# ningchungui/dbscan-on-spark

Measured on AMD Instinct MI355X. Metric: points clustered/sec (whole node) at 1/2/4/8 MI355X; % HBM roofline, higher is better.
Workload: dtype f64; 1 GPU; config 2: G(10000000 points, 32 Gaussian blobs, noise=0.0, dense=1.0, seed=1), eps=2.55, minPoints=10, LocalDBSCANNaive semantics; n_points=10000000, min_points=10, parallelism=single GPU, one local fit, world_size=1, clusters=14396, core_points=8854960, occupied_cells=1447458, occupied_tiles=44430

## Files before the change

dbscan-on-spark_amd/csrc/fit.hip:

```cpp
#include "internal.h"

#include <cmath>
#include <cstdio>
#include <cstdlib>
#include <cstring>
#include <vector>

namespace dbscan {

enum GridMode { kGridEps = 0, kGridAllPairs = 1, kGridNoPairs = 2 };

namespace {

constexpr int kTslot = 65;
constexpr int kQReg = 4;
constexpr int64_t kTileGrid = 8192;
constexpr int kMaxNbr = 11;
constexpr int32_t kModeArcheryBox = 2;
constexpr int64_t kBoxEdgeCap = 1 << 20;

#ifndef DBSCAN_AB_STAMPS
#define DBSCAN_AB_STAMPS 0
#endif
#if DBSCAN_AB_STAMPS
// ... 1319 lines not shown
                int ex = 0;
#pragma unroll
                for (int s = 4; s > 0; s >>= 1)
                    if (ex + s < 8 && st.off[base + ex + s] <= j) ex += s;
                const int p = st.cb[base + ex] + (j - st.off[base + ex]);
                const bool is_core =
                    min_points <= 0 || count_point<true>(st, buf, xy, cell, seg, j, r * 8 + ex, p,
                                                         eps2, min_points, lst, nbr, nbr_k);
                parent[p] = p;
                core[p] = is_core ? 1 : 0;
                mine += is_core ? 1 : 0;
            }
        } else {
            for (int p = st.ts + (int)threadIdx.x; p < st.te; p += kBlock) {
                const bool is_core =
                    min_points <= 0 || count_point<false>(st, buf, xy, cell, seg, 0, 0, p, eps2,
                                                          min_points, lst, nbr, nbr_k);
                parent[p] = p;
                core[p] = is_core ? 1 : 0;
                mine += is_core ? 1 : 0;
            }
        }
        __syncthreads();
    }
    for (int o = 32; o > 0; o >>= 1) mine += __shfl_xor(mine, o, 64);
    if (__lane_id() == 0) wcores[threadIdx.x >> 6] = mine;
    __syncthreads();
    if (threadIdx.x == 0) {
        int tot = 0;
        for (int w = 0; w < kBlock / 64; ++w) tot += wcores[w];
        block_cores[blockIdx.x] = tot;
    }
}

struct F32Cut {
    float lo, hi;
    float ne2;
};

__device__ __forceinline__ F32Cut f32_cut(const GridParams& g, double eps2) {
    const double s = 0.5 * g.invx;
    const double e2 = eps2 * s * s;
    return {__double2float_rd(e2 - 0x1p-14), __double2float_ru(e2 + 0x1p-14), -(float)e2};
}

constexpr float kCountBand = 0x1p-14f;
typedef float pk2f __attribute__((ext_vector_type(2)));
__device__ __forceinline__ float count_d(float2 me, float2 q, float ne2) {
    const pk2f d = pk2f{q.x, q.y} - pk2f{me.x, me.y};
    return __builtin_fmaf(d.x, d.x, __builtin_fmaf(d.y, d.y, ne2));
}

__device__ __forceinline__ int stage_slot(const TileStage& st, int q) {
    int k = 0;
#pragma unroll
    for (int s = 64; s > 0; s >>= 1)
        if (k + s < 100 && st.off[k + s] <= q) k += s;
    return st.cb[k] + (q - st.off[k]);
}

__device__ __forceinline__ float f32_d2(float2 a, float2 b) {
    const float dx = b.x - a.x, dy = b.y - a.y;
    return __builtin_fmaf(dx, dx, dy * dy);
}

template <int CAP>
__device__ bool stage_build32(const StageMeta& m, const double2* __restrict__ xy, TileStage& st,
                              float2* buf, const GridParams& g, const TileOrg& o) {
    const int tid = threadIdx.x;
    if (tid < 100) {
        st.cb[tid] = m.b;
        st.cn[tid] = m.cnt;
    }
    if (tid == 0) {
        st.ts = m.ts;
        st.te = m.te;
        st.q0 = m.q0;
        st.nq = m.q1 - m.q0;
    }
    __syncthreads();
    if (tid < 64) {
        int carry = 0;
        for (int base = 0; base < 100; base += 64) {
            const int i = base + tid;
            const int v = i < 100 ? st.cn[i] : 0;
            int incl = v;
#pragma unroll
            for (int o = 1; o < 64; o <<= 1) {
                const int u = __shfl_up(incl, o, 64);
                if (tid >= o) incl += u;
            }
            if (i < 100) st.off[i] = carry + incl - v;
            carry += __shfl(incl, 63, 64);
        }
        if (tid == 0) {
            st.off[100] = carry;
            st.total = carry;
            st.ok = carry <= CAP;
        }
    }
    __syncthreads();
    if (st.ok) {
        constexpr int kPer = (CAP + kBlock - 1) / kBlock;
        const int total = st.total;
#pragma unroll
        for (int u = 0; u < kPer; ++u) {
            const int i = tid + u * kBlock;
            if (i < total) {
                int lo = 0;
#pragma unroll
                for (int s = 64; s > 0; s >>= 1)
                    if (lo + s < 100 && st.off[lo + s] <= i) lo += s;
                const double2 v = xy[st.cb[lo] + (i - st.off[lo])];
                buf[i] = make_float2((float)((v.x * 0.5 - o.xmin2) * g.invx - o.ox),
                                     (float)((v.y * 0.5 - o.ymin2) * g.invy - o.oy));
            }
        }
    }
    __syncthreads();
    return st.ok;
}

template <class CoreF, class ExactF>
__device__ __forceinline__ bool quarters_touch32(const float2* __restrict__ buf, int ab, int ae,
                                                 uint32_t am, int bb, int be, uint32_t bm,
                                                 CoreF is_core, F32Cut cut, ExactF exact) {
    if (ae - ab <= 32 && be - bb <= 32) {
        for (uint32_t m1 = am; m1; m1 &= m1 - 1) {
            const int ia = ab + __ffs(m1) - 1;
            const float2 pa = buf[ia];
            for (uint32_t m2 = bm; m2; m2 &= m2 - 1) {
                const int ib = bb + __ffs(m2) - 1;
                const float F = f32_d2(pa, buf[ib]);
                if (F <= cut.lo) return true;
                if (F <= cut.hi && exact(ia, ib)) return true;
            }
        }
        return false;
    }
    for (int i = ab; i < ae; ++i) {
        if (!is_core(i)) continue;
        const float2 pa = buf[i];
        for (int j = bb; j < be; ++j) {
            if (!is_core(j)) continue;
            const float F = f32_d2(pa, buf[j]);
            if (F <= cut.lo) return true;
            if (F <= cut.hi && exact(i, j)) return true;
        }
    }
    return false;
}


template <class CoreF, class ExactF>
__device__ __forceinline__ void unite_adjacent32(int* lp, const uint32_t* lrange,
                                                 const uint32_t* lmask, const uint16_t* qmap,
                                                 int qi, const float2* __restrict__ buf,
                                                 CoreF is_core, F32Cut cut, ExactF exact) {
    constexpr int kDx[4] = {-1, 0, 1, -1}, kDy[4] = {-1, -1, -1, 0};
    const uint32_t ri = lrange[qi], am = lmask[qi];
    const int lq = (int)((ri >> 22) & 255u);
    const int ab = (int)(ri & 2047u), ae = ab + (int)((ri >> 11) & 2047u);
    int jn[4];
#pragma unroll
    for (int o = 0; o < 4; ++o) {
        const int ux = (lq & 15) + kDx[o], uy = (lq >> 4) + kDy[o];
        jn[o] = (ux >= 0 && ux <= 15 && uy >= 0) ? (int)qmap[uy * 16 + ux] : 0xFFFF;
    }
    uint32_t rj[4], mj[4];
#pragma unroll
    for (int o = 0; o < 4; ++o) {
        const int jj = jn[o] == 0xFFFF ? qi : jn[o];
        rj[o] = jn[o] == 0xFFFF ? 0u : lrange[jj];
        mj[o] = lmask[jj];
    }
    const float2 pa = buf[ab + (am ? __ffs(am) - 1 : 0)];
    bool t[4];
#pragma unroll
    for (int o = 0; o < 4; ++o) {
        const float2 pb = buf[(int)(rj[o] & 2047u) + (mj[o] ? __ffs(mj[o]) - 1 : 0)];
        t[o] = (rj[o] >> 31) && am && mj[o] && f32_d2(pa, pb) <= cut.lo;
    }
#pragma unroll
    for (int o = 0; o < 4; ++o) {
        if ((rj[o] >> 31) && !t[o]) {
            const int bb = (int)(rj[o] & 2047u), be = bb + (int)((rj[o] >> 11) & 2047u);
            t[o] = quarters_touch32(buf, ab, ae, am, bb, be, mj[o], is_core, cut, exact);
        }
        if (t[o]) lunite(lp, qi, jn[o]);
    }
}

constexpr int kScanBatch = 4;
template <bool REC, int STRIDE = kBlock, class ExactF>
__device__ __forceinline__ bool scan_count32(const float2* __restrict__ buf, int b, int e,
                                             float2 me, F32Cut cut, int min_points, int& cnt,
                                             uint32_t* lst, int& nrec, int nbr_k, int tag,
                                             ExactF exact, int* nbatch = nullptr) {
    for (int j = b; j < e; j += kScanBatch) {
        if (nbatch) ++*nbatch;
        const int nin = e - j;
        float2 qq[kScanBatch];
#pragma unroll
        for (int u = 0; u < kScanBatch; ++u) qq[u] = buf[j + u];
        const uint32_t valid = nin >= kScanBatch ? (1u << kScanBatch) - 1u : (1u << nin) - 1u;
        uint32_t hm = 0, am = 0;
        float d[kScanBatch];
#pragma unroll
        for (int u = 0; u < kScanBatch; ++u) d[u] = count_d(me, qq[u], cut.ne2);
#pragma unroll
        for (int u = kScanBatch - 1; u >= 0; --u)
            hm = __builtin_amdgcn_alignbit(hm, __float_as_uint(d[u]), 31);
        hm &= valid;
        float mn = fabsf(d[0]);
#pragma unroll
        for (int u = 1; u < kScanBatch; ++u) mn = fminf(mn, fabsf(d[u]));
        if (__builtin_expect(mn <= kCountBand, 0)) {
#pragma unroll
            for (int u = 0; u < kScanBatch; ++u)
                if (((valid >> u) & 1u) && fabsf(d[u]) <= kCountBand) am |= 1u << u;
            hm &= ~am;
        }
        if (__builtin_expect(am != 0, 0)) {
            for (uint32_t m = am; m; m &= m - 1) {
                const int u = __ffs(m) - 1;
                if (exact(j + u)) hm |= 1u << u;
            }
        }
        if (REC && hm && nrec < nbr_k) {
            lst[nrec * STRIDE] = (uint32_t)j | ((uint32_t)tag << 11) | (hm << 16);
            ++nrec;
        }
        cnt += __popc(hm);
        if (cnt >= min_points) return true;
    }
    return cnt >= min_points;
}

__device__ void fused_tile_union32(int t, int q0, int nq, int b, int e, uint32_t key,
                                   const FuseArgs& fa,
                                   const GridParams& g, const TileStage& st,
                                   const float2* __restrict__ buf,
                                   const uint32_t* __restrict__ lcore,
                                   const double2* __restrict__ xy, double eps2, F32Cut cut,
                                   int32_t* __restrict__ parent, UnionLds& u) {
    const int i = threadIdx.x;
    const auto is_core = [&](int j) { return ((lcore[j >> 5] >> (j & 31)) & 1u) != 0; };
    const auto exact = [&](int qa, int qb) {
        const double2 pa = xy[stage_slot(st, qa)], pb = xy[stage_slot(st, qb)];
        return within_eps(pa.x, pa.y, pb.x, pb.y, eps2);
    };
    __shared__ int s_first;
    __shared__ int s_tflags;
    if (i == 0) {
        s_first = 0x7FFFFFFF;
        s_tflags = 0;
    }
    u.qmap[i] = 0xFFFF;
    u.cmin[i] = ~0ull;
    lds_barrier();
    int rep = -1, best = 0x7FFFFFFF, gx = 0, gy = 0;
    if (i < nq) {
        uint32_t cx, cy;
        cell_xy(key >> 2, g.ntx, cx, cy);
        gx = (int)(2 * cx + (key & 1u));
        gy = (int)(2 * cy + ((key >> 1) & 1u));
        const int lq = (gy & 15) * 16 + (gx & 15);
        const int len = e - b;
        const int l = (int)((key >> 2) & 63u);
        const int k = ((l >> 3) + 1) * 10 + (l & 7) + 1;
        const int jb = st.off[k] + (b - st.cb[k]);
        uint32_t mask = 0;
        int first = -1;
        if (len <= 32) {
            const int w = jb >> 5, o = jb & 31;
            const uint64_t v = (uint64_t)lcore[w] | ((uint64_t)lcore[w + 1] << 32);
            mask = (uint32_t)(v >> o) & (len == 32 ? ~0u : ((1u << len) - 1u));
            first = mask ? __ffs(mask) - 1 : -1;
        } else {
            for (int j = 0; j < len && (j < 32 || first < 0); ++j)
                if (is_core(jb + j)) {
                    if (j < 32) mask |= 1u << j;
                    if (first < 0) first = j;
                }
        }
        if (first >= 0) {
            rep = b + first;
            best = fa.perm[rep];
        }
        if (rep >= 0) {
            atomicMin(&s_first, i);
            const int tf = ((gx & 15) >= 14 ? 1 : 0) | ((gy & 15) >= 14 ? 2 : 0);
            if (tf) atomicOr(&s_tflags, tf);
        }
        fa.qinfo[q0 + i] = make_int4(b, e, rep, (int)mask);
        u.lp[i] = i;
        u.lrange[i] = (rep >= 0 ? 0x80000000u : 0u) | ((uint32_t)lq << 22) | (uint32_t)jb |
                      ((uint32_t)len << 11);
        u.lmask[i] = mask;
        u.qmap[lq] = (uint16_t)i;
    }
    lds_barrier();
    if (i == 0) fa.tcore[t] = (uint8_t)s_tflags;
    AB_STAMP(5);
    {
        if (i < nq && rep >= 0)
            unite_adjacent32(u.lp, u.lrange, u.lmask, u.qmap, i, buf, is_core, cut, exact);
        lds_barrier();
        AB_STAMP(6);
        const int f = s_first;
        const bool split = i < nq && rep >= 0 && lfind(u.lp, i) != lfind(u.lp, f);
        if (__syncthreads_or(split)) {
            for (int k = i; k < nq * 8; k += kBlock) {
                const int o = k / nq, qi = k - o * nq;
                const uint32_t ri = u.lrange[qi];
                if (!(ri >> 31)) continue;
                const int lq = (int)((ri >> 22) & 255u);
                const int ux = (lq & 15) + kRingDx[4 + o], uy = (lq >> 4) + kRingDy[4 + o];
                if (ux < 0 || uy < 0 || ux > 15 || uy > 15) continue;
                const int j = u.qmap[uy * 16 + ux];
                if (j == 0xFFFF) continue;
                const uint32_t rj = u.lrange[j];
                if (!(rj >> 31)) continue;
                if (lfind(u.lp, qi) == lfind(u.lp, j)) continue;
                const int ab = (int)(ri & 2047u), ae = ab + (int)((ri >> 11) & 2047u);
                const int bb = (int)(rj & 2047u), be = bb + (int)((rj >> 11) & 2047u);
                if (quarters_touch32(buf, ab, ae, u.lmask[qi], bb, be, u.lmask[j], is_core, cut,
                                     exact))
                    lunite(u.lp, qi, j);
            }
            lds_barrier();
        }
        AB_STAMP(7);
    }
    int r = -1;
    if (i < nq && rep >= 0) {
        r = lfind(u.lp, i);
        atomicMin(&u.cmin[r], ((unsigned long long)(uint32_t)best << 32) | (uint32_t)rep);
    }
    lds_barrier();
    AB_STAMP(8);
    if (i < nq) {
        const int crep = r >= 0 ? (int)(uint32_t)(u.cmin[r] & 0xFFFFFFFFull) : -1;
        fa.qg[q0 + i] = make_int4(gx, gy, best, 0);
        fa.qcomp[q0 + i] = crep;
        if (rep >= 0) parent[rep] = crep;
    }
}

template <int CAP, int MINW>
__global__ __launch_bounds__(kBlock, MINW) void count_tile32_kernel(
    const double2* __restrict__ xy, const int32_t* __restrict__ tstart,
    const int2* __restrict__ tstage, const int32_t* __restrict__ ntiles_p, double eps2,
    int32_t min_points, uint8_t* __restrict__ core, int32_t* __restrict__ parent,
    int32_t* __restrict__ block_cores, int32_t* __restrict__ nbr, int nbr_k, FuseArgs fa) {
    const GridParams g = *fa.gp;
    if (!g.clique) {
        if (threadIdx.x == 0) block_cores[blockIdx.x] = 0;
        return;
    }
    __shared__ TileStage st;
    __shared__ float2 buf[CAP + kScanBatch];
    __shared__ int wcores[kBlock / 64];
    __shared__ int rowoff[9];
    __shared__ __attribute__((aligned(16))) uint32_t lsts[kMaxNbr * kBlock];
    __shared__ uint32_t lcore[(CAP + 31) / 32 + 1];
    static_assert(CAP < 2048, "LDS ranges are packed in 11 bits");
    static_assert(sizeof(UnionLds) <= sizeof(lsts), "UnionLds must fit");
    uint32_t* lst = lsts + threadIdx.x;
    const int ntiles = *ntiles_p;
    const F32Cut cut = f32_cut(g, eps2);
    int mine = 0;
    const BucketWalk<kMedBuckets> order(fa.tl.mb);
    const int nt = order.size();
    const auto tile_at = [&](int k) { return k < nt ? order.at(fa.tl.medium, fa.tl.cap, k) : ntiles; };
    StageMeta meta = stage_meta(tile_at(blockIdx.x), ntiles, tstage, tstart, fa.tq);
    for (int k = blockIdx.x; k < nt; k += gridDim.x) {
        AB_STAMP(0);
        const int t = tile_at(k);
        if (threadIdx.x < (CAP + 31) / 32 + 1) lcore[threadIdx.x] = 0u;
        stage_build32<CAP>(meta, xy, st, buf, g, tile_org(g, fa.tpart, t, fa.tkey[t]));
        AB_STAMP(1);
        AB_NOTE(10, st.total);
        meta = stage_meta(tile_at(k + gridDim.x), ntiles, tstage, tstart, fa.tq);
        const int q0 = st.q0, nq = st.nq;
        int qb = 0, qe = 0;
        uint32_t qk = 0;
        if ((int)threadIdx.x < nq) {
            qb = fa.qstart[q0 + threadIdx.x];
            qe = fa.qstart[q0 + threadIdx.x + 1];
            qk = fa.qkey[q0 + threadIdx.x];
        }
        {
            if (threadIdx.x == 0) {
                int acc = 0;
                for (int r = 0; r < 8; ++r) {
                    rowoff[r] = acc;
                    acc += st.off[(r + 1) * 10 + 9] - st.off[(r + 1) * 10 + 1];
                }
                rowoff[8] = acc;
            }
            __syncthreads();
            AB_STAMP(2);
            const int own = rowoff[8];
            AB_NOTE(11, own);
            for (int i = (int)threadIdx.x; i < own; i += kBlock) {
                int r = 0;
#pragma unroll
                for (int s = 4; s > 0; s >>= 1)
                    if (r + s < 8 && rowoff[r + s] <= i) r += s;
                const int base = (r + 1) * 10 + 1;
                const int j = st.off[base] + (i - rowoff[r]);
                int ex = 0;
#pragma unroll
                for (int s = 4; s > 0; s >>= 1)
                    if (ex + s < 8 && st.off[base + ex + s] <= j) ex += s;
                const int p = st.cb[base + ex] + (j - st.off[base + ex]);
                bool is_core = true;
                if (min_points > 0) {
                    const int l = r * 8 + ex;
                    const float2 me = buf[j];
                    const LdsRanges rg = lds_ranges(st, l);
                    const auto exact = [&](int q) {
                        const double2 a = xy[p], o = xy[stage_slot(st, q)];
                        return within_eps(a.x, a.y, o.x, o.y, eps2);
                    };
                    int cnt = 0, nrec = 0;
                    const int k_rec = nbr_k;
#if DBSCAN_AB_COUNTDIV
                    int nbt = 0;
                    int* const nbp = &nbt;
#else
                    int* const nbp = nullptr;
#endif
                    bool done = scan_count32<true>(buf, rg.cs, rg.ce, me, cut, min_points, cnt,
                                                   lst, nrec, k_rec, 0, exact, nbp);
#pragma unroll
                    for (int k = 0; k < 3 && !done; ++k) {
                        const int lo = rg.b[k], hi = rg.e[k];
                        if (lo <= rg.cs && rg.ce <= hi) {
                            done = scan_count32<true>(buf, lo, rg.cs, me, cut, min_points, cnt,
                                                      lst, nrec, k_rec, k, exact, nbp) ||
                                   scan_count32<true>(buf, rg.ce, hi, me, cut, min_points, cnt,
                                                      lst, nrec, k_rec, k, exact, nbp);
                        } else {
                            done = scan_count32<true>(buf, lo, hi, me, cut, min_points, cnt, lst,
                                                      nrec, k_rec, k, exact, nbp);
                        }
                    }
                    is_core = cnt >= min_points;
#if DBSCAN_AB_COUNTDIV
                    {
                        const uint64_t act = __ballot(1);
                        int mx = nbt, sm = nbt;
                        for (int o = 32; o > 0; o >>= 1) {
                            mx = max(mx, __shfl_xor(mx, o, 64));
                            sm += __shfl_xor(sm, o, 64);
                        }
                        const uint64_t cm = __ballot(is_core);
                        if (__lane_id() == __builtin_ctzll(act)) {
                            atomicAdd(&g_div[0], (unsigned long long)mx);
                            atomicAdd(&g_div[1], (unsigned long long)sm);
                            atomicAdd(&g_div[2], (unsigned long long)__popcll(act));
                            atomicAdd(&g_div[3], (unsigned long long)__popcll(cm));
                            atomicAdd(&g_div[4], 1ull);
                        }
                    }
#endif
                    if (!is_core && k_rec > 0) {
                        int32_t* out = nbr + (int64_t)p * nbr_k;
                        int w = 0;
                        for (int rr = 0; rr < nrec; ++rr) {
                            const uint32_t v = lst[rr * kBlock];
                            const int q = (int)(v & 2047u), row = (int)((v >> 11) & 3u);
                            const int k0 = (r + (row == 0 ? 0 : (row == 1 ? -1 : 1)) + 1) * 10 + ex;
                            for (uint32_t m = v >> 16; m; m &= m - 1) {
                                const int qq = q + __ffs(m) - 1;
                                const int c = k0 + (qq >= st.off[k0 + 1] ? 1 : 0) +
                                              (qq >= st.off[k0 + 2] ? 1 : 0);
                                const int sq = st.cb[c] + (qq - st.off[c]);
                                if (sq != p) out[w++] = sq;
                            }
                        }
                        if (w < nbr_k) out[w] = -1;
                    }
                }
                if (fa.zs && fa.zs[p] == 2) is_core = false;
                if (is_core) atomicOr(&lcore[j >> 5], 1u << (j & 31));
                core[p] = is_core ? 1 : 0;
                mine += is_core ? 1 : 0;
            }
            AB_STAMP(3);
            __syncthreads();
            AB_STAMP(4);
            fused_tile_union32(t, q0, nq, qb, qe, qk, fa, g, st, buf, lcore, xy, eps2, cut, parent,
                               *reinterpret_cast<UnionLds*>(lsts));
        }
        __syncthreads();
        AB_STAMP(9);
    }
    for (int o = 32; o > 0; o >>= 1) mine += __shfl_xor(mine, o, 64);
    if (__lane_id() == 0) wcores[threadIdx.x >> 6] = mine;
    __syncthreads();
    if (threadIdx.x == 0) {
        int tot = 0;
        for (int w = 0; w < kBlock / 64; ++w) tot += wcores[w];
        block_cores[blockIdx.x] = tot;
    }
}


template <int SCAP>
struct WaveUnion {
    int lp[SCAP];
    uint32_t lrange[SCAP];
    uint32_t lmask[SCAP];
    unsigned long long cmin[SCAP];
    uint16_t qmap[kMaxTileQ];
};

template <int SCAP>
struct WaveSeg {
    TileStage st;
    int rowoff[9];
    uint32_t lcore[SCAP / 32 + 1];
    float2 buf[SCAP + kScanBatch];
};

template <int SCAP, int NSEG>
struct WaveTile {
    WaveSeg<SCAP> sg[NSEG];
    union {
        uint32_t rec[kMaxNbr * 64];
        WaveUnion<SCAP> u[NSEG];
    };
};

template <int MINW, int SEG, int SCAP, int B0, int NB, int WAVES>
__global__ __launch_bounds__(64 * WAVES, MINW) void count_wave_kernel(
    const double2* __restrict__ xy, const int32_t* __restrict__ tstart,
    const int2* __restrict__ tstage, double eps2, int32_t min_points,
    uint8_t* __restrict__ core, int32_t* __restrict__ parent,
    int32_t* __restrict__ block_cores, int32_t* __restrict__ nbr, int nbr_k, FuseArgs fa) {
    constexpr int NSEG = 64 / SEG, NQ = SCAP / SEG;
    static_assert(B0 + NB <= kSmallBuckets && 64 % SEG == 0 && SEG >= 8 && SCAP % SEG == 0,
                  "small-tile buckets / segments");
    __shared__ WaveTile<SCAP, NSEG> wt[WAVES];
    __shared__ int wcores[WAVES];
    const GridParams g = *fa.gp;
    const int lane = __lane_id(), w = threadIdx.x >> 6;
    const int sgi = lane / SEG, sl = lane - sgi * SEG;
    const uint64_t smask = SEG == 64 ? ~0ull : (((1ull << SEG) - 1) << (sgi * SEG));
    WaveSeg<SCAP>& T = wt[w].sg[sgi];
    TileStage& st = T.st;
    WaveUnion<SCAP>& u = wt[w].u[sgi];
    int mine = 0;
    if (g.clique) {
        const F32Cut cut = f32_cut(g, eps2);
        const BucketWalk<NB> order(fa.tl.sb + B0);
        const int32_t* lists = fa.tl.small + (int64_t)B0 * fa.tl.cap;
        const int nt = order.size();
        const int ngroups = (nt + NSEG - 1) / NSEG;
        for (int kg = blockIdx.x * WAVES + w; kg < ngroups; kg += gridDim.x * WAVES) {
            const int k = kg * NSEG + sgi;
            const bool live = k < nt;
            const int t = live ? order.at(lists, fa.tl.cap, k) : 0;
            constexpr int kRounds = (100 + SEG - 1) / SEG;
            int2 m[kRounds];
#pragma unroll
            for (int r = 0; r < kRounds; ++r) {
                const int e = r * SEG + sl;
                m[r] = (live && e < 100) ? tstage[(int64_t)t * 100 + e] : make_int2(0, 0);
            }
            const uint32_t tk = live ? fa.tkey[t] : 0u;
            const int q0 = live ? fa.tq[(int64_t)t * kTslot] : 0;
            const int nq = live ? fa.tq[(int64_t)t * kTslot + 64] - q0 : 0;
            int incl[kRounds];
#pragma unroll
            for (int r = 0; r < kRounds; ++r) incl[r] = m[r].y;
#pragma unroll
            for (int o = 1; o < SEG; o <<= 1) {
#pragma unroll
                for (int r = 0; r < kRounds; ++r) {
                    const int v = __shfl_up(incl[r], o, SEG);
                    if (sl >= o) incl[r] += v;
                }
            }
            int carry = 0;
#pragma unroll
            for (int r = 0; r < kRounds; ++r) {
                const int e = r * SEG + sl;
                if (e < 100) {
                    st.cb[e] = m[r].x;
                    st.off[e] = carry + incl[r] - m[r].y;
                }
                carry += __shfl(incl[r], SEG - 1, SEG);
            }
            const int total = carry;
            if (sl == 0) st.off[100] = total;
            if (sl < SCAP / 32 + 1) T.lcore[sl] = 0u;
            wave_sync();
            {
                const TileOrg o = live ? tile_org(g, fa.tpart, t, tk) : TileOrg{0, 0, 0, 0};
#pragma unroll
                for (int uu = 0; uu < SCAP / SEG; ++uu) {
                    const int e = sl + uu * SEG;
                    if (e < total) {
                        int c = 0;
#pragma unroll
                        for (int sh = 64; sh > 0; sh >>= 1)
                            if (c + sh < 100 && st.off[c + sh] <= e) c += sh;
                        const double2 v = xy[st.cb[c] + (e - st.off[c])];
                        T.buf[e] = make_float2((float)((v.x * 0.5 - o.xmin2) * g.invx - o.ox),
                                               (float)((v.y * 0.5 - o.ymin2) * g.invy - o.oy));
                    }
                }
            }
            if (sl < 8) {
                const int rs = st.off[(sl + 1) * 10 + 9] - st.off[(sl + 1) * 10 + 1];
                int rincl = rs;
#pragma unroll
                for (int o = 1; o < 8; o <<= 1) {
                    const int v = __shfl_up(rincl, o, SEG);
                    if (sl >= o) rincl += v;
                }
                T.rowoff[sl] = rincl - rs;
                if (sl == 7) T.rowoff[8] = rincl;
            }
            wave_sync();
            const int own = T.rowoff[8];
            int tflags = 0;
            for (int i = sl; i < own; i += SEG) {
                int r = 0;
#pragma unroll
                for (int sh = 4; sh > 0; sh >>= 1)
                    if (r + sh < 8 && T.rowoff[r + sh] <= i) r += sh;
                const int base = (r + 1) * 10 + 1;
                const int j = st.off[base] + (i - T.rowoff[r]);
                int ex = 0;
#pragma unroll
                for (int sh = 4; sh > 0; sh >>= 1)
                    if (ex + sh < 8 && st.off[base + ex + sh] <= j) ex += sh;
                const int p = st.cb[base + ex] + (j - st.off[base + ex]);
                bool is_core = true;
                if (min_points > 0) {
                    const float2 me = T.buf[j];
                    const LdsRanges rg = lds_ranges(st, r * 8 + ex);
                    const auto exact = [&](int q) {
                        const double2 a = xy[p], o = xy[stage_slot(st, q)];
                        return within_eps(a.x, a.y, o.x, o.y, eps2);
                    };
                    uint32_t* lst = wt[w].rec + lane;
                    int cnt = 0, nrec = 0;
                    bool done = scan_count32<true, 64>(T.buf, rg.cs, rg.ce, me, cut, min_points,
                                                       cnt, lst, nrec, nbr_k, 0, exact);
#pragma unroll
                    for (int kk = 0; kk < 3 && !done; ++kk) {
                        const int lo = rg.b[kk], hi = rg.e[kk];
                        if (lo <= rg.cs && rg.ce <= hi) {
                            done = scan_count32<true, 64>(T.buf, lo, rg.cs, me, cut, min_points,
                                                          cnt, lst, nrec, nbr_k, kk, exact) ||
                                   scan_count32<true, 64>(T.buf, rg.ce, hi, me, cut, min_points,
                                                          cnt, lst, nrec, nbr_k, kk, exact);
                        } else {
                            done = scan_count32<true, 64>(T.buf, lo, hi, me, cut, min_points, cnt,
                                                          lst, nrec, nbr_k, kk, exact);
                        }
                    }
                    is_core = cnt >= min_points;
                    if (!is_core && nbr_k > 0) {
                        int32_t* out = nbr + (int64_t)p * nbr_k;
                        int wn = 0;
                        for (int rr = 0; rr < nrec; ++rr) {
                            const uint32_t v = lst[rr * 64];
                            const int q = (int)(v & 2047u), row = (int)((v >> 11) & 3u);
                            const int k0 = (r + (row == 0 ? 0 : (row == 1 ? -1 : 1)) + 1) * 10 + ex;
                            for (uint32_t mm = v >> 16; mm; mm &= mm - 1) {
                                const int qq = q + __ffs(mm) - 1;
                                const int c = k0 + (qq >= st.off[k0 + 1] ? 1 : 0) +
                                              (qq >= st.off[k0 + 2] ? 1 : 0);
                                const int sq = st.cb[c] + (qq - st.off[c]);
                                if (sq != p) out[wn++] = sq;
                            }
                        }
                        if (wn < nbr_k) out[wn] = -1;
                    }
                }
                if (fa.zs && fa.zs[p] == 2) is_core = false;
                if (is_core) atomicOr(&T.lcore[j >> 5], 1u << (j & 31));
                if (is_core) tflags |= (ex == 7 ? 1 : 0) | (r == 7 ? 2 : 0);
                core[p] = is_core ? 1 : 0;
                mine += is_core ? 1 : 0;
            }
            {
                const uint64_t b0 = __ballot(tflags & 1) & smask, b1 = __ballot(tflags & 2) & smask;
                if (live && sl == 0) fa.tcore[t] = (uint8_t)((b0 ? 1 : 0) | (b1 ? 2 : 0));
            }
            wave_sync();
            for (int idx = sl; idx < kMaxTileQ; idx += SEG) u.qmap[idx] = 0xFFFF;
            for (int idx = sl; idx < SCAP; idx += SEG) u.cmin[idx] = ~0ull;
            wave_sync();
            int rep[NQ], best[NQ];
#pragma unroll
            for (int pp = 0; pp < NQ; ++pp) {
                const int qi = sl + pp * SEG;
                rep[pp] = -1;
                best[pp] = 0x7FFFFFFF;
                if (qi < nq) {
                    const int b = fa.qstart[q0 + qi], e = fa.qstart[q0 + qi + 1];
                    const uint32_t key = fa.qkey[q0 + qi];
                    uint32_t cx, cy;
                    cell_xy(key >> 2, g.ntx, cx, cy);
                    const int gx = (int)(2 * cx + (key & 1u)), gy = (int)(2 * cy + ((key >> 1) & 1u));
                    const int lq = (gy & 15) * 16 + (gx & 15);
                    const int len = e - b;
                    const int l = (int)((key >> 2) & 63u);
                    const int kc = ((l >> 3) + 1) * 10 + (l & 7) + 1;
                    const int jb = st.off[kc] + (b - st.cb[kc]);
                    uint32_t mask = 0;
                    int first = -1;
                    for (int jj = 0; jj < len && (jj < 32 || first < 0); ++jj)
                        if ((T.lcore[(jb + jj) >> 5] >> ((jb + jj) & 31)) & 1u) {
                            if (jj < 32) mask |= 1u << jj;
                            if (first < 0) first = jj;
                        }
                    if (first >= 0) {
                        rep[pp] = b + first;
                        best[pp] = fa.perm[rep[pp]];
                    }
                    fa.qinfo[q0 + qi] = make_int4(b, e, rep[pp], (int)mask);
                    fa.qg[q0 + qi] = make_int4(gx, gy, best[pp], 0);
                    u.lp[qi] = qi;
                    u.lrange[qi] = (rep[pp] >= 0 ? 0x80000000u : 0u) | ((uint32_t)lq << 22) |
                                   (uint32_t)jb | ((uint32_t)len << 11);
                    u.lmask[qi] = mask;
                    u.qmap[lq] = (uint16_t)qi;
                }
            }
            wave_sync();
            const auto is_core_l = [&](int j) { return ((T.lcore[j >> 5] >> (j & 31)) & 1u) != 0; };
            const auto exact2 = [&](int qa, int qb) {
                const double2 pa = xy[stage_slot(st, qa)], pb = xy[stage_slot(st, qb)];
                return within_eps(pa.x, pa.y, pb.x, pb.y, eps2);
            };
            for (int qi = sl; qi < nq; qi += SEG)
                if (u.lrange[qi] >> 31)
                    unite_adjacent32(u.lp, u.lrange, u.lmask, u.qmap, qi, T.buf, is_core_l, cut,
                                     exact2);
            wave_sync();
            int f = 0x7FFFFFFF;
#pragma unroll
            for (int pp = NQ - 1; pp >= 0; --pp)
                if (sl + pp * SEG < nq && rep[pp] >= 0) f = sl + pp * SEG;
#pragma unroll
            for (int o = SEG / 2; o > 0; o >>= 1) f = min(f, __shfl_xor(f, o, SEG));
            bool split = false;
#pragma unroll
            for (int pp = 0; pp < NQ; ++pp) {
                const int qi = sl + pp * SEG;
                if (qi < nq && rep[pp] >= 0 && lfind(u.lp, qi) != lfind(u.lp, f)) split = true;
            }
            if (__ballot(split) & smask) {
                wave_sync();
                for (int it = sl; it < nq * 8; it += SEG) {
                    const int o = it / nq, qi = it - o * nq;
                    const uint32_t ri = u.lrange[qi];
                    if (!(ri >> 31)) continue;
                    const int lq = (int)((ri >> 22) & 255u);
                    const int ux = (lq & 15) + kRingDx[4 + o], uy = (lq >> 4) + kRingDy[4 + o];
                    if (ux < 0 || uy < 0 || ux > 15 || uy > 15) continue;
                    const int j = u.qmap[uy * 16 + ux];
                    if (j == 0xFFFF) continue;
                    const uint32_t rj = u.lrange[j];
                    if (!(rj >> 31)) continue;
                    if (lfind(u.lp, qi) == lfind(u.lp, j)) continue;
                    const int ab = (int)(ri & 2047u), ae = ab + (int)((ri >> 11) & 2047u);
                    const int bb = (int)(rj & 2047u), be = bb + (int)((rj >> 11) & 2047u);
                    if (quarters_touch32(T.buf, ab, ae, u.lmask[qi], bb, be, u.lmask[j],
                                         is_core_l, cut, exact2))
                        lunite(u.lp, qi, j);
                }
            }
            wave_sync();
            int rr[NQ];
#pragma unroll
            for (int pp = 0; pp < NQ; ++pp) {
                const int qi = sl + pp * SEG;
                rr[pp] = -1;
                if (qi < nq && rep[pp] >= 0) {
                    rr[pp] = lfind(u.lp, qi);
                    atomicMin(&u.cmin[rr[pp]],
                              ((unsigned long long)(uint32_t)best[pp] << 32) | (uint32_t)rep[pp]);
                }
            }
            wave_sync();
#pragma unroll
            for (int pp = 0; pp < NQ; ++pp) {
                const int qi = sl + pp * SEG;
                if (qi < nq) {
                    const int crep =
                        rr[pp] >= 0 ? (int)(uint32_t)(u.cmin[rr[pp]] & 0xFFFFFFFFull) : -1;
                    fa.qcomp[q0 + qi] = crep;
                    if (rep[pp] >= 0) parent[rep[pp]] = crep;
                }
            }
            wave_sync();
        }
    }
    for (int o = 32; o > 0; o >>= 1) mine += __shfl_xor(mine, o, 64);
    if (lane == 0) wcores[w] = mine;
    __syncthreads();
    if (threadIdx.x == 0) {
        int tot = 0;
        for (int v = 0; v < WAVES; ++v) tot += wcores[v];
        block_cores[blockIdx.x] = tot;
    }
}

constexpr int kBigChunks = 8;
template <int MINW, int WAVES>
__global__ __launch_bounds__(64 * WAVES, MINW) void big_count_kernel(
    const double2* __restrict__ xy, const int32_t* __restrict__ cell,
    const Seg* __restrict__ seg, const int32_t* __restrict__ tstart,
    const int32_t* __restrict__ qidx, double eps2, int32_t min_points,
    uint8_t* __restrict__ core, int32_t* __restrict__ block_cores, int32_t* __restrict__ nbr,
    int nbr_k, FuseArgs fa) {
    constexpr int CS = 64 * WAVES, NC = kBigChunks * kBlock / CS;
    __shared__ int wcores[WAVES];
    __shared__ TileStage st;
    int mine = 0;
    if (fa.gp->clique) {
        const int nb = fa.tl.n[kTileBig];
        for (int k = blockIdx.x; k < nb * NC; k += gridDim.x) {
            const int t = fa.tl.big[k / NC], c = k % NC;
            const int te = tstart[t + 1];
            for (int p = tstart[t] + c * CS + (int)threadIdx.x; p < te;
                 p += kBigChunks * kBlock) {
                const int q = qidx[p];
                const int lb = fa.qstart[q + 1] - fa.qstart[q];
                const bool is_core =
                    (min_points <= 0 || lb >= min_points ||
                     count_point<false>(st, nullptr, xy, cell, seg, 0, 0, p, eps2, min_points,
                                        nullptr, nbr, nbr_k)) &&
                    !(fa.zs && fa.zs[p] == 2);
                core[p] = is_core ? 1 : 0;
                mine += is_core ? 1 : 0;
            }
        }
    }
    for (int o = 32; o > 0; o >>= 1) mine += __shfl_xor(mine, o, 64);
    if (__lane_id() == 0) wcores[threadIdx.x >> 6] = mine;
    __syncthreads();
    if (threadIdx.x == 0) {
        int tot = 0;
        for (int w = 0; w < WAVES; ++w) tot += wcores[w];
        block_cores[blockIdx.x] = tot;
    }
}

__global__ __launch_bounds__(kBlock) void big_union_kernel(const double2* __restrict__ xy,
                                                           const uint8_t* __restrict__ core,
                                                           double eps2,
                                                           int32_t* __restrict__ parent,
                                                           FuseArgs fa) {
    const GridParams g = *fa.gp;
    if (!g.clique) return;
    __shared__ UnionLds u;
    const int nb = fa.tl.n[kTileBig];
    for (int k = blockIdx.x; k < nb; k += gridDim.x) {
        const int t = fa.tl.big[k];
        const int q0 = fa.tq[(int64_t)t * kTslot], nq = fa.tq[(int64_t)t * kTslot + 64] - q0;
        int qb = 0, qe = 0;
        uint32_t qk = 0;
        if ((int)threadIdx.x < nq) {
            qb = fa.qstart[q0 + threadIdx.x];
            qe = fa.qstart[q0 + threadIdx.x + 1];
            qk = fa.qkey[q0 + threadIdx.x];
        }
        global_tile_union(q0, nq, qb, qe, qk, fa, g, xy, core, eps2, parent, u);
        __syncthreads();
    }
}

__global__ __launch_bounds__(kBlock) void zone_fix_kernel(int64_t n,
                                                          const uint8_t* __restrict__ zone,
                                                          const int32_t* __restrict__ inv,
                                                          uint8_t* __restrict__ core) {
    const int64_t i = (int64_t)blockIdx.x * kBlock + threadIdx.x;
    if (i < n && zone[i] == 2) core[inv[i]] = 0;
}

__global__ __launch_bounds__(kBlock) void zone_fix_sorted_kernel(int64_t n,
                                                                 const uint8_t* __restrict__ zs,
                                                                 uint8_t* __restrict__ core) {
    const int64_t p = (int64_t)blockIdx.x * kBlock + threadIdx.x;
    if (p < n && zs[p] == 2) core[p] = 0;
}

__global__ __launch_bounds__(kBlock) void count_rest_kernel(const int32_t* __restrict__ nf_p,
                                                            int64_t n,
                                                            int32_t min_points,
                                                            uint8_t* __restrict__ core,
                                                            int32_t* __restrict__ parent,
                                                            int32_t* __restrict__ block_cores) {
    count_rest_body(blockIdx.x, gridDim.x, nf_p, n, min_points, core, parent, block_cores);
}

template <int V>
__device__ __forceinline__ int ld_par(int* par, int i) {
    if constexpr (V == 1) {
        return par[i];
    } else {
        return __hip_atomic_load(par + i, __ATOMIC_RELAXED, __HIP_MEMORY_SCOPE_AGENT);
    }
}
__device__ __forceinline__ void st_par(int* par, int i, int v) {
    __hip_atomic_store(par + i, v, __ATOMIC_RELAXED, __HIP_MEMORY_SCOPE_AGENT);
}

template <int V = 0>
__device__ int uf_find(int* par, int x) {
    int cur = ld_par<V>(par, x);
    if (cur == x) return x;
    int prev = x;
    for (;;) {
        const int next = ld_par<V>(par, cur);
        if (next == cur) return cur;
        if constexpr (V == 0) st_par(par, prev, next);
        prev = cur;
        cur = next;
    }
}

template <int V = 0>
__device__ int uf_find_until(int* par, int x, int target) {
    if (x == target) return target;
    int cur = ld_par<V>(par, x);
    if (cur == x || cur == target) return cur;
    int prev = x;
    for (;;) {
        const int next = ld_par<V>(par, cur);
        if (next == cur || next == target) return next;
        if constexpr (V == 0) st_par(par, prev, next);
        prev = cur;
        cur = next;
    }
}
// ... 1783 lines not shown
```

Before: 6.470 billion points/s.

## Replace per-tile lock-based union-find with adjacency bitmask label propagation

Tile-local connectivity no longer uses lunite/lfind pointer chasing. Each quarter pair is now tested once and the hit is recorded as a bit in an adjacency mask. Components are then found with hook-and-compress label propagation that runs either across the whole block or per wave segment, and that propagation is skipped when the tile has a single component. The wave path also shrinks its LDS footprint by storing qmap as bytes and overlapping the cmin and adj arrays in a union. The aim is to cut serialized find chains and redundant pair checks, at the cost of extra barrier rounds when a tile has many components.

New measurement: 6.553 billion points/s, median of 6. Within noise of the previous version (+1.3%).

```diff
diff --git a/dbscan-on-spark_amd/csrc/fit.hip b/dbscan-on-spark_amd/csrc/fit.hip
--- a/dbscan-on-spark_amd/csrc/fit.hip
+++ b/dbscan-on-spark_amd/csrc/fit.hip
@@ -1495,43 +1495,162 @@
 }
 
 
-template <class CoreF, class ExactF>
-__device__ __forceinline__ void unite_adjacent32(int* lp, const uint32_t* lrange,
-                                                 const uint32_t* lmask, const uint16_t* qmap,
-                                                 int qi, const float2* __restrict__ buf,
-                                                 CoreF is_core, F32Cut cut, ExactF exact) {
-    constexpr int kDx[4] = {-1, 0, 1, -1}, kDy[4] = {-1, -1, -1, 0};
-    const uint32_t ri = lrange[qi], am = lmask[qi];
+constexpr int kRingDxC[12] = {-1, 0, 1, -1, -2, -1, 0, 1, 2, -2, 2, -2};
+constexpr int kRingDyC[12] = {-1, -1, -1, 0, -2, -2, -2, -2, -2, -1, -1, 0};
+constexpr uint64_t kRingDxLut = 0x040432101321ull, kRingDyLut = 0x211000002111ull;
+constexpr bool ring_luts_match() {
+    for (int o = 0; o < 12; ++o)
+        if ((int)((kRingDxLut >> (4 * o)) & 15u) - 2 != kRingDxC[o] ||
+            (int)((kRingDyLut >> (4 * o)) & 15u) - 2 != kRingDyC[o])
+            return false;
+    return true;
+}
+static_assert(ring_luts_match(), "kRingDxLut / kRingDyLut restate kRingDx / kRingDy");
+
+template <class QMapT>
+__device__ __forceinline__ int ring_far_end(const QMapT* qmap, int lq, int o) {
+    return (int)qmap[lq + (int)((kRingDxLut >> (4 * o)) & 15u) - 2 +
+                     16 * ((int)((kRingDyLut >> (4 * o)) & 15u) - 2)];
+}
+
+template <int SH, class QMapT, class CoreF, class ExactF>
+__device__ __forceinline__ bool tile_pair_item(uint32_t* adj, const uint32_t* lrange,
+                                               const uint32_t* lmask, const QMapT* qmap,
+                                               const int* labels, int k,
+                                               const float2* __restrict__ buf, CoreF is_core,
+                                               F32Cut cut, ExactF exact) {
+    const int qi = k >> SH, o = SH == 2 ? (k & 3) : 4 + (k & 7);
+    const uint32_t ri = lrange[qi];
+    if (!(ri >> 31)) return false;
     const int lq = (int)((ri >> 22) & 255u);
+    const int ux = (lq & 15) + (int)((kRingDxLut >> (4 * o)) & 15u) - 2;
+    const int uy = (lq >> 4) + (int)((kRingDyLut >> (4 * o)) & 15u) - 2;
+    if (ux < 0 || ux > 15 || uy < 0) return false;
+    const int j = (int)qmap[uy * 16 + ux];
+    if (j == (int)(QMapT)~0u) return false;
+    const uint32_t rj = lrange[j];
+    if (!(rj >> 31)) return false;
+    if (labels && labels[qi] == labels[j]) return false;
+    const uint32_t am = lmask[qi], bm = lmask[j];
     const int ab = (int)(ri & 2047u), ae = ab + (int)((ri >> 11) & 2047u);
-    int jn[4];
-#pragma unroll
-    for (int o = 0; o < 4; ++o) {
-        const int ux = (lq & 15) + kDx[o], uy = (lq >> 4) + kDy[o];
-        jn[o] = (ux >= 0 && ux <= 15 && uy >= 0) ? (int)qmap[uy * 16 + ux] : 0xFFFF;
-    }
-    uint32_t rj[4], mj[4];
-#pragma unroll
-    for (int o = 0; o < 4; ++o) {
-        const int jj = jn[o] == 0xFFFF ? qi : jn[o];
-        rj[o] = jn[o] == 0xFFFF ? 0u : lrange[jj];
-        mj[o] = lmask[jj];
-    }
-    const float2 pa = buf[ab + (am ? __ffs(am) - 1 : 0)];
-    bool t[4];
-#pragma unroll
-    for (int o = 0; o < 4; ++o) {
-        const float2 pb = buf[(int)(rj[o] & 2047u) + (mj[o] ? __ffs(mj[o]) - 1 : 0)];
-        t[o] = (rj[o] >> 31) && am && mj[o] && f32_d2(pa, pb) <= cut.lo;
-    }
-#pragma unroll
-    for (int o = 0; o < 4; ++o) {
-        if ((rj[o] >> 31) && !t[o]) {
-            const int bb = (int)(rj[o] & 2047u), be = bb + (int)((rj[o] >> 11) & 2047u);
-            t[o] = quarters_touch32(buf, ab, ae, am, bb, be, mj[o], is_core, cut, exact);
-        }
-        if (t[o]) lunite(lp, qi, jn[o]);
-    }
+    const int bb = (int)(rj & 2047u), be = bb + (int)((rj >> 11) & 2047u);
+    bool t = false;
+    if (am && bm) t = f32_d2(buf[ab + __ffs(am) - 1], buf[bb + __ffs(bm) - 1]) <= cut.lo;
+    if (!t) t = quarters_touch32(buf, ab, ae, am, bb, be, bm, is_core, cut, exact);
+    if (t) atomicOr(&adj[qi], 1u << o);
+    return t;
+}
+
+struct BlockSteps {
+    int* s;
+    int k = 0;
+    __device__ __forceinline__ void sync() { lds_barrier(); }
+    __device__ __forceinline__ int sum(int v) {
+        const int slot = k % 3;
+        const uint64_t b = __ballot(v != 0);
+        if (b && __lane_id() == __builtin_ctzll(b)) atomicAdd(&s[slot], __popcll(b));
+        if (threadIdx.x == 0) s[(k + 1) % 3] = 0;
+        lds_barrier();
+        ++k;
+        return s[slot];
+    }
+};
+template <int SEG>
+struct SegSteps {
+    __device__ __forceinline__ void sync() { wave_sync(); }
+    __device__ __forceinline__ int sum(int v) {
+        wave_sync();
+#pragma unroll
+        for (int o = SEG / 2; o > 0; o >>= 1) v += __shfl_xor(v, o, SEG);
+        return v;
+    }
+};
+
+__device__ __forceinline__ int label_load(int* p) {
+    return __hip_atomic_load(p, __ATOMIC_RELAXED, __HIP_MEMORY_SCOPE_WORKGROUP);
+}
+
+template <int NQ, int STRIDE, class Steps>
+__device__ __forceinline__ void tile_compress(Steps& st, int q, int nq, int* labels) {
+    for (int trip = 0; trip < 8; ++trip) {
+        int g[NQ];
+        int moved = 0;
+#pragma unroll
+        for (int pp = 0; pp < NQ; ++pp) {
+            const int qi = q + pp * STRIDE;
+            g[pp] = 0;
+            if (qi < nq) {
+                const int p = labels[qi];
+                g[pp] = labels[p];
+                moved |= g[pp] != p ? 1 : 0;
+            }
+        }
+        st.sync();
+#pragma unroll
+        for (int pp = 0; pp < NQ; ++pp)
+            if (q + pp * STRIDE < nq) labels[q + pp * STRIDE] = g[pp];
+        if (!st.sum(moved)) break;
+    }
+}
+
+template <int NQ, int STRIDE, class Steps, class QMapT>
+__device__ __forceinline__ void tile_hook(Steps& st, int q, int nq, const uint32_t* lrange,
+                                          const QMapT* qmap, const uint32_t* adj, int* labels,
+                                          uint32_t bits) {
+    for (int trip = 0; trip < kMaxTileQ; ++trip) {
+        int hooked = 0;
+#pragma unroll
+        for (int pp = 0; pp < NQ; ++pp) {
+            const int qi = q + pp * STRIDE;
+            uint32_t a = qi < nq ? adj[qi] & bits : 0u;
+            if (!a) continue;
+            const int lq = (int)((lrange[qi] >> 22) & 255u);
+            const int ru = label_load(&labels[qi]);
+            for (; a; a &= a - 1) {
+                const int rv = label_load(&labels[ring_far_end(qmap, lq, __ffs(a) - 1)]);
+                if (ru != rv) {
+                    atomicMin(&labels[max(ru, rv)], min(ru, rv));
+                    hooked = 1;
+                }
+            }
+        }
+        if (!st.sum(hooked)) break;
+        tile_compress<NQ, STRIDE>(st, q, nq, labels);
+    }
+}
+
+template <int NQ, int STRIDE, class Steps, class QMapT>
+__device__ __forceinline__ int tile_components(Steps& st, int q, int nq, const uint32_t* lrange,
+                                               const QMapT* qmap, const uint32_t* adj,
+                                               int* labels) {
+    uint32_t a[NQ];
+    bool core[NQ];
+    int roots = 0;
+#pragma unroll
+    for (int pp = 0; pp < NQ; ++pp) {
+        const int qi = q + pp * STRIDE;
+        core[pp] = qi < nq && (lrange[qi] >> 31);
+        a[pp] = core[pp] ? adj[qi] & 15u : 0u;
+        roots += core[pp] && !a[pp] ? 1 : 0;
+    }
+    const int nroots = st.sum(roots);
+    if (nroots <= 1) return nroots;
+#pragma unroll
+    for (int pp = 0; pp < NQ; ++pp) {
+        const int qi = q + pp * STRIDE;
+        if (qi < nq)
+            labels[qi] = a[pp] ? ring_far_end(qmap, (int)((lrange[qi] >> 22) & 255u),
+                                              __ffs(a[pp]) - 1)
+                               : qi;
+    }
+    st.sync();
+    tile_compress<NQ, STRIDE>(st, q, nq, labels);
+    tile_hook<NQ, STRIDE>(st, q, nq, lrange, qmap, adj, labels, 15u);
+    int own = 0;
+#pragma unroll
+    for (int pp = 0; pp < NQ; ++pp)
+        own += core[pp] && labels[q + pp * STRIDE] == q + pp * STRIDE ? 1 : 0;
+    return st.sum(own);
 }
 
 constexpr int kScanBatch = 4;
@@ -1580,27 +1699,36 @@
     return cnt >= min_points;
 }
 
+struct UnionLds32 {
+    uint32_t lrange[kMaxTileQ];
+    uint32_t lmask[kMaxTileQ];
+    uint16_t qmap[kMaxTileQ];
+    uint32_t adj[kMaxTileQ];
+    int labels[kMaxTileQ];
+    unsigned long long cmin[kMaxTileQ];
+};
+
 __device__ void fused_tile_union32(int t, int q0, int nq, int b, int e, uint32_t key,
                                    const FuseArgs& fa,
                                    const GridParams& g, const TileStage& st,
                                    const float2* __restrict__ buf,
                                    const uint32_t* __restrict__ lcore,
                                    const double2* __restrict__ xy, double eps2, F32Cut cut,
-                                   int32_t* __restrict__ parent, UnionLds& u) {
-    const int i = threadIdx.x;
+                                   int32_t* __restrict__ parent, UnionLds32& u) {
+    int i = threadIdx.x;
+    asm volatile("" : "+v"(i));
     const auto is_core = [&](int j) { return ((lcore[j >> 5] >> (j & 31)) & 1u) != 0; };
     const auto exact = [&](int qa, int qb) {
         const double2 pa = xy[stage_slot(st, qa)], pb = xy[stage_slot(st, qb)];
         return within_eps(pa.x, pa.y, pb.x, pb.y, eps2);
     };
-    __shared__ int s_first;
     __shared__ int s_tflags;
-    if (i == 0) {
-        s_first = 0x7FFFFFFF;
-        s_tflags = 0;
-    }
+    __shared__ int s_steps[3];
+    if (i == 0) s_tflags = 0;
+    if (i < 3) s_steps[i] = 0;
     u.qmap[i] = 0xFFFF;
     u.cmin[i] = ~0ull;
+    u.adj[i] = 0u;
     lds_barrier();
     int rep = -1, best = 0x7FFFFFFF, gx = 0, gy = 0;
     if (i < nq) {
@@ -1632,12 +1760,10 @@
             best = fa.perm[rep];
         }
         if (rep >= 0) {
-            atomicMin(&s_first, i);
             const int tf = ((gx & 15) >= 14 ? 1 : 0) | ((gy & 15) >= 14 ? 2 : 0);
             if (tf) atomicOr(&s_tflags, tf);
         }
         fa.qinfo[q0 + i] = make_int4(b, e, rep, (int)mask);
-        u.lp[i] = i;
         u.lrange[i] = (rep >= 0 ? 0x80000000u : 0u) | ((uint32_t)lq << 22) | (uint32_t)jb |
                       ((uint32_t)len << 11);
         u.lmask[i] = mask;
@@ -1646,39 +1772,26 @@
     lds_barrier();
     if (i == 0) fa.tcore[t] = (uint8_t)s_tflags;
     AB_STAMP(5);
-    {
-        if (i < nq && rep >= 0)
-            unite_adjacent32(u.lp, u.lrange, u.lmask, u.qmap, i, buf, is_core, cut, exact);
-        lds_barrier();
-        AB_STAMP(6);
-        const int f = s_first;
-        const bool split = i < nq && rep >= 0 && lfind(u.lp, i) != lfind(u.lp, f);
-        if (__syncthreads_or(split)) {
-            for (int k = i; k < nq * 8; k += kBlock) {
-                const int o = k / nq, qi = k - o * nq;
-                const uint32_t ri = u.lrange[qi];
-                if (!(ri >> 31)) continue;
-                const int lq = (int)((ri >> 22) & 255u);
-                const int ux = (lq & 15) + kRingDx[4 + o], uy = (lq >> 4) + kRingDy[4 + o];
-                if (ux < 0 || uy < 0 || ux > 15 || uy > 15) continue;
-                const int j = u.qmap[uy * 16 + ux];
-                if (j == 0xFFFF) continue;
-                const uint32_t rj = u.lrange[j];
-                if (!(rj >> 31)) continue;
-                if (lfind(u.lp, qi) == lfind(u.lp, j)) continue;
-                const int ab = (int)(ri & 2047u), ae = ab + (int)((ri >> 11) & 2047u);
-                const int bb = (int)(rj & 2047u), be = bb + (int)((rj >> 11) & 2047u);
-                if (quarters_touch32(buf, ab, ae, u.lmask[qi], bb, be, u.lmask[j], is_core, cut,
-                                     exact))
-                    lunite(u.lp, qi, j);
-            }
-            lds_barrier();
-        }
-        AB_STAMP(7);
-    }
+    BlockSteps steps{s_steps};
+    for (int k = i; k < nq * 4; k += kBlock)
+        tile_pair_item<2>(u.adj, u.lrange, u.lmask, u.qmap, nullptr, k, buf, is_core, cut, exact);
+    lds_barrier();
+    const int ncomp = tile_components<1, kBlock>(steps, i, nq, u.lrange, u.qmap, u.adj, u.labels);
+    AB_STAMP(6);
+    if (ncomp > 1) {
+        int hit = 0;
+        for (int k = i; k < nq * 8; k += kBlock)
+            hit |= tile_pair_item<3>(u.adj, u.lrange, u.lmask, u.qmap, u.labels, k, buf, is_core,
+                                     cut, exact)
+                       ? 1
+                       : 0;
+        if (steps.sum(hit))
+            tile_hook<1, kBlock>(steps, i, nq, u.lrange, u.qmap, u.adj, u.labels, 0xFF0u);
+    }
+    AB_STAMP(7);
     int r = -1;
     if (i < nq && rep >= 0) {
-        r = lfind(u.lp, i);
+        r = ncomp == 1 ? 0 : u.labels[i];
         atomicMin(&u.cmin[r], ((unsigned long long)(uint32_t)best << 32) | (uint32_t)rep);
     }
     lds_barrier();
@@ -1709,7 +1822,7 @@
     __shared__ __attribute__((aligned(16))) uint32_t lsts[kMaxNbr * kBlock];
     __shared__ uint32_t lcore[(CAP + 31) / 32 + 1];
     static_assert(CAP < 2048, "LDS ranges are packed in 11 bits");
-    static_assert(sizeof(UnionLds) <= sizeof(lsts), "UnionLds must fit");
+    static_assert(sizeof(UnionLds32) <= sizeof(lsts), "UnionLds32 must fit");
     uint32_t* lst = lsts + threadIdx.x;
     const int ntiles = *ntiles_p;
     const F32Cut cut = f32_cut(g, eps2);
@@ -1837,7 +1950,7 @@
             __syncthreads();
             AB_STAMP(4);
             fused_tile_union32(t, q0, nq, qb, qe, qk, fa, g, st, buf, lcore, xy, eps2, cut, parent,
-                               *reinterpret_cast<UnionLds*>(lsts));
+                               *reinterpret_cast<UnionLds32*>(lsts));
         }
         __syncthreads();
         AB_STAMP(9);
@@ -1855,12 +1968,19 @@
 
 template <int SCAP>
 struct WaveUnion {
-    int lp[SCAP];
+    union {
+        unsigned long long cmin[SCAP];
+        uint32_t adj[SCAP];
+    };
     uint32_t lrange[SCAP];
     uint32_t lmask[SCAP];
-    unsigned long long cmin[SCAP];
-    uint16_t qmap[kMaxTileQ];
+    int labels[SCAP];
+    uint8_t qmap[kMaxTileQ];
+    static_assert(SCAP < 255, "quarter indices and the empty mark fit a byte");
 };
+static_assert(sizeof(WaveUnion<kSmallCap>) <= 20 * kSmallCap + 2 * kMaxTileQ &&
+                  sizeof(WaveUnion<kTinyCap>) <= 20 * kTinyCap + 2 * kMaxTileQ + 64,
+              "WaveUnion grew");
 
 template <int SCAP>
 struct WaveSeg {
@@ -2040,8 +2160,8 @@
                 if (live && sl == 0) fa.tcore[t] = (uint8_t)((b0 ? 1 : 0) | (b1 ? 2 : 0));
             }
             wave_sync();
-            for (int idx = sl; idx < kMaxTileQ; idx += SEG) u.qmap[idx] = 0xFFFF;
-            for (int idx = sl; idx < SCAP; idx += SEG) u.cmin[idx] = ~0ull;
+            for (int idx = sl; idx < kMaxTileQ; idx += SEG) u.qmap[idx] = 0xFF;
+            for (int idx = sl; idx < SCAP; idx += SEG) u.adj[idx] = 0u;
             wave_sync();
             int rep[NQ], best[NQ];
 #pragma unroll
@@ -2073,11 +2193,10 @@
                     }
                     fa.qinfo[q0 + qi] = make_int4(b, e, rep[pp], (int)mask);
                     fa.qg[q0 + qi] = make_int4(gx, gy, best[pp], 0);
-                    u.lp[qi] = qi;
                     u.lrange[qi] = (rep[pp] >= 0 ? 0x80000000u : 0u) | ((uint32_t)lq << 22) |
                                    (uint32_t)jb | ((uint32_t)len << 11);
                     u.lmask[qi] = mask;
-                    u.qmap[lq] = (uint16_t)qi;
+                    u.qmap[lq] = (uint8_t)qi;
                 }
             }
             wave_sync();
@@ -2086,56 +2205,38 @@
                 const double2 pa = xy[stage_slot(st, qa)], pb = xy[stage_slot(st, qb)];
                 return within_eps(pa.x, pa.y, pb.x, pb.y, eps2);
             };
-            for (int qi = sl; qi < nq; qi += SEG)
-                if (u.lrange[qi] >> 31)
-                    unite_adjacent32(u.lp, u.lrange, u.lmask, u.qmap, qi, T.buf, is_core_l, cut,
-                                     exact2);
+            SegSteps<SEG> steps;
+            for (int k = sl; k < nq * 4; k += SEG)
+                tile_pair_item<2>(u.adj, u.lrange, u.lmask, u.qmap, nullptr, k, T.buf, is_core_l,
+                                  cut, exact2);
             wave_sync();
-            int f = 0x7FFFFFFF;
-#pragma unroll
-            for (int pp = NQ - 1; pp >= 0; --pp)
-                if (sl + pp * SEG < nq && rep[pp] >= 0) f = sl + pp * SEG;
-#pragma unroll
-            for (int o = SEG / 2; o > 0; o >>= 1) f = min(f, __shfl_xor(f, o, SEG));
-            bool split = false;
-#pragma unroll
-            for (int pp = 0; pp < NQ; ++pp) {
-                const int qi = sl + pp * SEG;
-                if (qi < nq && rep[pp] >= 0 && lfind(u.lp, qi) != lfind(u.lp, f)) split = true;
-            }
-            if (__ballot(split) & smask) {
-                wave_sync();
-                for (int it = sl; it < nq * 8; it += SEG) {
-                    const int o = it / nq, qi = it - o * nq;
-                    const uint32_t ri = u.lrange[qi];
-                    if (!(ri >> 31)) continue;
-                    const int lq = (int)((ri >> 22) & 255u);
-                    const int ux = (lq & 15) + kRingDx[4 + o], uy = (lq >> 4) + kRingDy[4 + o];
-                    if (ux < 0 || uy < 0 || ux > 15 || uy > 15) continue;
-                    const int j = u.qmap[uy * 16 + ux];
-                    if (j == 0xFFFF) continue;
-                    const uint32_t rj = u.lrange[j];
-                    if (!(rj >> 31)) continue;
-                    if (lfind(u.lp, qi) == lfind(u.lp, j)) continue;
-                    const int ab = (int)(ri & 2047u), ae = ab + (int)((ri >> 11) & 2047u);
-                    const int bb = (int)(rj & 2047u), be = bb + (int)((rj >> 11) & 2047u);
-                    if (quarters_touch32(T.buf, ab, ae, u.lmask[qi], bb, be, u.lmask[j],
-                                         is_core_l, cut, exact2))
-                        lunite(u.lp, qi, j);
-                }
-            }
-            wave_sync();
+            const int ncomp =
+                tile_components<NQ, SEG>(steps, sl, nq, u.lrange, u.qmap, u.adj, u.labels);
+            if (ncomp > 1) {
+                int hit = 0;
+                for (int k = sl; k < nq * 8; k += SEG)
+                    hit |= tile_pair_item<3>(u.adj, u.lrange, u.lmask, u.qmap, u.labels, k, T.buf,
+                                             is_core_l, cut, exact2)
+                               ? 1
+                               : 0;
+                if (steps.sum(hit))
+                    tile_hook<NQ, SEG>(steps, sl, nq, u.lrange, u.qmap, u.adj, u.labels, 0xFF0u);
+            }
             int rr[NQ];
 #pragma unroll
             for (int pp = 0; pp < NQ; ++pp) {
                 const int qi = sl + pp * SEG;
                 rr[pp] = -1;
-                if (qi < nq && rep[pp] >= 0) {
-                    rr[pp] = lfind(u.lp, qi);
+                if (qi < nq && rep[pp] >= 0) rr[pp] = ncomp == 1 ? 0 : u.labels[qi];
+            }
+            wave_sync();
+            for (int idx = sl; idx < SCAP; idx += SEG) u.cmin[idx] = ~0ull;
+            wave_sync();
+#pragma unroll
+            for (int pp = 0; pp < NQ; ++pp)
+                if (rr[pp] >= 0)
                     atomicMin(&u.cmin[rr[pp]],
                               ((unsigned long long)(uint32_t)best[pp] << 32) | (uint32_t)rep[pp]);
-                }
-            }
             wave_sync();
 #pragma unroll
             for (int pp = 0; pp < NQ; ++pp) {
```
